# rasmusab/bayes.js

Measured on AMD Instinct MI355X. Metric: posterior draws/sec (= param-updates/sec), higher is better.
Workload: dtype f64

## Files before the change

### bayes.js_amd/csrc/amwg_models.h

```cpp
#pragma once
#include "amwg_div.h"
#include "amwg_ld.h"
#include "amwg_pass.h"
#include "amwg_twoval.h"
#include "amwg_types.h"
#include "amwg_window.h"

namespace amwg {

__device__ __forceinline__ double norm_const_sd(double v, double m, double c_sd, double den, double y_hi, double y_lo, int den_ok) {
  const double t = v - m;
  const double tt = t * t;
  const double q = (den_ok && wide_range(tt)) ? div_by_invariant(tt, den, Reciprocal{y_hi, y_lo}) : tt / den;
  return c_sd - q;
}

struct NormCache {
  double sd, c, den;
  Reciprocal y;
  bool den_ok;
};
__device__ __forceinline__ NormCache norm_cache_init() { return NormCache{__builtin_nan(""), 0.0, 0.0, Reciprocal{0.0, 0.0}, false}; }
AMWG_HD NormCache norm_cache_make(double sd, double neg_half_log_2pi) {
  NormCache k;
  k.sd = sd;
  k.c = norm_c(neg_half_log_2pi, sd);
  k.den = norm_den(sd);
  k.y = make_reciprocal(k.den);
  k.den_ok = mid_range(k.den);
  return k;
}
struct NormCacheA { double c, den; };
AMWG_HD_OUTLINE NormCacheA norm_cache_cold_a(double sd, double neg_half_log_2pi) { return NormCacheA{norm_c(neg_half_log_2pi, sd), norm_den(sd)}; }
AMWG_HD_OUTLINE Reciprocal norm_cache_cold_b(double den) { return make_reciprocal(den); }
template <bool COLD = false>
__device__ __forceinline__ void norm_cache_update(NormCache &k, double sd, double neg_half_log_2pi) {
  if (sd != k.sd) {
    if constexpr (COLD) {
      const NormCacheA a = norm_cache_cold_a(sd, neg_half_log_2pi);
      k.sd = sd; k.c = a.c; k.den = a.den;
      k.y = norm_cache_cold_b(a.den);
      k.den_ok = mid_range(a.den);
    } else {
      k = norm_cache_make(sd, neg_half_log_2pi);
    }
  }
}



struct NormalModel {
  static constexpr bool kSplitPrior = false;
  static constexpr bool kUser = false, kHasFast = true, kOneLanePass = false;
  static constexpr int kDerived = 0;
  static constexpr bool kHasBinary = false;
  static constexpr int kMaxThreads = 1024;
  static constexpr int kUnroll = 8;
  struct Pass { double mu, c, den; Reciprocal y; bool fast; const double *x; };
  static constexpr size_t kOneLaneTileLimit = 96 * 1024;
  __host__ __device__ static size_t one_lane_tile_bytes(int n_obs) { return (size_t)n_obs * 8 <= kOneLaneTileLimit ? (size_t)n_obs * 8 : 0; }
  __host__ __device__ static size_t lds_bytes(int n_obs, int, int lanes) { return lanes == 1 ? 0 : (size_t)n_obs * 8; }
  static constexpr bool kDynamicLds = true;
  __host__ __device__ static size_t lds_bytes_of(const DataRef &d, int lanes, int) { return lanes == 1 ? (d.pad > 0 ? one_lane_tile_bytes(d.n_obs) : 0) : (size_t)d.n_obs * 8; }
  __device__ static void stage(unsigned char *smem, const DataRef &d, int tid, int nt, int lanes) {
    if (lanes == 1 && lds_bytes_of(d, 1, nt) == 0) return;
    double *dst = reinterpret_cast<double *>(smem);
    for (int i = tid; i < d.n_obs; i += nt) dst[i] = d.x[i];
  }
  template <class C>
  __device__ __forceinline__ static double prior(const StateView &, const ModelConsts &mc, const DataRef &, C &kc) {
    double lp = 0;
    lp += norm_const_sd(kc.mu, mc.m0, mc.c0, mc.den0, mc.y0_hi, mc.y0_lo, mc.den0_ok);
    const double sigma = kc.sigma;
    lp += (sigma < mc.ua || sigma > mc.ub) ? -kInf : mc.lunif;
    return lp;
  }
  static constexpr bool kTracksState = true;
  struct Cache { NormCache n; double mu, sigma; bool loaded; };
  __device__ __forceinline__ static Cache cache_init() { return Cache{norm_cache_init(), 0.0, 0.0, false}; }
  __device__ __forceinline__ static void on_set(Cache &k, int comp, double v, int, const DataRef &) { k.mu = comp == 0 ? v : k.mu; k.sigma = comp == 0 ? k.sigma : v; }
  static constexpr bool kMirrorCheck = true;
  template <int GL>
  __device__ __forceinline__ static bool mirror_ok(const Cache &k, const StateView &S, const DataRef &, int) {
    return !k.loaded || (f64_bits(k.mu) == f64_bits(S(0)) && f64_bits(k.sigma) == f64_bits(S(1)));
  }
  template <int GL>
  __device__ __forceinline__ static void load(Cache &k, const StateView &S, const ModelConsts &, const DataRef &, const unsigned char *, int) {
    if (!k.loaded) { k.mu = S(0); k.sigma = S(1); k.loaded = true; }
  }
  template <int GL>
  __device__ __forceinline__ static Pass begin(const StateView &, const ModelConsts &mc, const DataRef &d,
                                               const unsigned char *smem, Cache &kc) {
    Pass ps;
    NormCache &k = kc.n;
    ps.mu = kc.mu;
    norm_cache_update(k, kc.sigma, mc.neg_half_log_2pi);
    ps.c = k.c;
    ps.den = k.den;
    ps.y = k.y;
    ps.fast = !mc.exact_division && mc.data_mid_range && k.den_ok &&
              (ps.mu == 0 || mid_range(__builtin_fabs(ps.mu)));
    ps.x = GL == 1 ? d.x : reinterpret_cast<const double *>(smem);
    return ps;
  }
  template <bool FAST>
  __device__ __forceinline__ static double term(const Pass &ps, int i) {
    const double t = ps.x[i] - ps.mu;
    const double tt = t * t;
    return ps.c - (FAST ? div_by_invariant(tt, ps.den, ps.y) : tt / ps.den);
  }
  template <int G>
  __device__ inline __attribute__((noinline)) static double pass_slow_impl(const double *x, double mu, double c, double den, int n_obs, int sub, double acc) {
    for (int i = sub; i < n_obs; i += G) { const double t = x[i] - mu; acc += c - (t * t) / den; }
    return acc;
  }
  template <int G>
  __device__ __forceinline__ static double pass_slow(const Pass &ps, int n_obs, int sub, double acc) { return pass_slow_impl<G>(ps.x, ps.mu, ps.c, ps.den, n_obs, sub, acc); }
  static constexpr bool kStagedFast = true;
  template <int G, int U = 8>
  __device__ __forceinline__ static double pass_fast(const Pass &ps, int n_obs, int sub, double acc) {
    if constexpr (G == 1) return norm_pass_uniform<8>(ps.x, ps.mu, ps.c, ps.den, ps.y, n_obs, acc);
    else return norm_pass_staged<G, U, false>(ps.x, nullptr, StateView{nullptr}, ps.mu, ps.c, ps.den, ps.y, n_obs, sub, acc);
  }
  static constexpr bool kCertified = true;
  static constexpr int kCertifiedLanes = 1;
  struct Approx { double value, eps; };
  template <int G, int BT>
  __device__ __forceinline__ static Approx log_post_approx(Cache &kc, const StateView &S, const ModelConsts &mc, const DataRef &d, const unsigned char *smem, int sub) {
    static_assert(G == 1, "the certified pass of the Normal family is the one-lane one");
    load<G>(kc, S, mc, d, smem, sub);
    norm_cache_update(kc.n, kc.sigma, mc.neg_half_log_2pi);
    const double P = prior(S, mc, d, kc);
    double S2;
    if (mc.sufficient) {
      const double dm = (mc.suff_xbar_hi - kc.mu) + mc.suff_xbar_lo;
      S2 = __builtin_fma((double)d.n_obs, dm * dm, mc.suff_ss);
    } else
    if constexpr (BT <= 512) S2 = norm_sq_pass_wave<(BT <= 256 ? kWaveBlock : 8)>(lds_bytes_of(d, 1, 0) ? reinterpret_cast<const double *>(smem) : d.x, kc.mu, d.n_obs, wave_scratch_of(d));
    else S2 = norm_sq_pass_uniform<8>(d.x, kc.mu, d.n_obs);
    const double n = (double)d.n_obs;
    const double Q = S2 * kc.n.y.hi, nc = n * kc.n.c;
    const double mag = __builtin_fabs(P) + __builtin_fabs(nc) + 2.0 * Q;
    return Approx{(P + nc) - Q, (2.0 * n + 64.0) * 0x1p-53 * mag * 1.25};
  }
};

struct BetaBernModel {
  static constexpr bool kSplitPrior = false;
  static constexpr bool kUser = false, kHasFast = false, kOneLanePass = true;
  static constexpr int kDerived = 0;
  static constexpr bool kHasBinary = false;
  static constexpr int kMaxThreads = 1024;
  static constexpr int kUnroll = 8;
  struct Pass { double l1, l0; const uint8_t *x; const uint32_t *bits; bool has_invalid, fast_forward; BitData B; };
  __host__ __device__ static size_t words(int n_obs) { return (size_t)n_obs / 32 + 2; }
  static constexpr size_t kFfLdsLimit = 120 * 1024;
  __host__ __device__ static size_t lds_bytes(int n_obs, int, int lanes) {
    if (lanes == 1) { const size_t b = 6 * words(n_obs) * 4; return b <= kFfLdsLimit ? ((b + 15) & ~(size_t)15) : 0; }
    return ((size_t)n_obs + 15) & ~(size_t)15;
  }
  __device__ static void stage(unsigned char *smem, const DataRef &d, int tid, int nt, int lanes) {
    if (lanes == 1) {
      if (lds_bytes(d.n_obs, 0, 1) == 0) return;
      uint32_t *dst = reinterpret_cast<uint32_t *>(smem);
      const uint32_t *src = static_cast<const uint32_t *>(d.arr[0]);
      for (int k = tid; k < (int)(6 * words(d.n_obs)); k += nt) dst[k] = src[k];
      return;
    }
    for (int i = tid; i < d.n_obs; i += nt) smem[i] = d.xb[i];
  }
  template <class C>
  __device__ __forceinline__ static double prior(const StateView &S, const ModelConsts &mc, const DataRef &, C &) {
    const double th = S(0);
    double lp = 0;
    if (th > 1 || th < 0) lp += -kInf;
    else if (mc.ba == 1 && mc.bb == 1) lp += 0.0;
    else lp += (mc.ba - 1) * log_v8(th) + (mc.bb - 1) * log_v8(1 - th) - mc.lbeta_ab;
    return lp;
  }
  struct Cache {};
  __device__ __forceinline__ static Cache cache_init() { return Cache{}; }
  template <int GL>
  __device__ __forceinline__ static Pass begin(const StateView &S, const ModelConsts &mc, const DataRef &d,
                                               const unsigned char *smem, Cache &) {
    Pass ps;
    const double th = S(0);
    ps.l1 = log_v8(th);
    ps.l0 = log_v8(1 - th);
    ps.x = smem;
    ps.bits = d.xw;
    ps.has_invalid = mc.has_invalid != 0;
    ps.fast_forward = !mc.exact_division;
    {
      const size_t W = words(d.n_obs);
      const uint32_t *base = lds_bytes(d.n_obs, 0, 1) ? reinterpret_cast<const uint32_t *>(smem) : static_cast<const uint32_t *>(d.arr[0]);
      ps.B.w = base; ps.B.pre = base + W; ps.B.om1 = base + 2 * W; ps.B.po1 = base + 3 * W; ps.B.om0 = base + 4 * W; ps.B.po0 = base + 5 * W;
      ps.B.n = d.n_obs;
    }
    return ps;
  }
  template <bool FAST>
  __device__ __forceinline__ static double term(const Pass &ps, int i) { return ps.x[i] ? ps.l1 : ps.l0; }

#define AMWG_A0 "v_add_f64 %[acc], %[acc], %[l0]\n"
#define AMWG_A1 "v_add_f64 %[acc], %[acc], %[l1]\n"
#define AMWG_N0 AMWG_A0 AMWG_A0 AMWG_A0 AMWG_A0
#define AMWG_N1 AMWG_A1 AMWG_A0 AMWG_A0 AMWG_A0
#define AMWG_N2 AMWG_A0 AMWG_A1 AMWG_A0 AMWG_A0
#define AMWG_N3 AMWG_A1 AMWG_A1 AMWG_A0 AMWG_A0
#define AMWG_N4 AMWG_A0 AMWG_A0 AMWG_A1 AMWG_A0
#define AMWG_N5 AMWG_A1 AMWG_A0 AMWG_A1 AMWG_A0
#define AMWG_N6 AMWG_A0 AMWG_A1 AMWG_A1 AMWG_A0
#define AMWG_N7 AMWG_A1 AMWG_A1 AMWG_A1 AMWG_A0
#define AMWG_N8 AMWG_A0 AMWG_A0 AMWG_A0 AMWG_A1
#define AMWG_N9 AMWG_A1 AMWG_A0 AMWG_A0 AMWG_A1
#define AMWG_N10 AMWG_A0 AMWG_A1 AMWG_A0 AMWG_A1
#define AMWG_N11 AMWG_A1 AMWG_A1 AMWG_A0 AMWG_A1
#define AMWG_N12 AMWG_A0 AMWG_A0 AMWG_A1 AMWG_A1
#define AMWG_N13 AMWG_A1 AMWG_A0 AMWG_A1 AMWG_A1
#define AMWG_N14 AMWG_A0 AMWG_A1 AMWG_A1 AMWG_A1
#define AMWG_N15 AMWG_A1 AMWG_A1 AMWG_A1 AMWG_A1
#define AMWG_B(HI, LO) AMWG_N##LO AMWG_N##HI "s_branch 25b\n"
#define AMWG_ROW(HI)                                                                                   \
  AMWG_B(HI, 0) AMWG_B(HI, 1) AMWG_B(HI, 2) AMWG_B(HI, 3) AMWG_B(HI, 4) AMWG_B(HI, 5) AMWG_B(HI, 6) AMWG_B(HI, 7) \
  AMWG_B(HI, 8) AMWG_B(HI, 9) AMWG_B(HI, 10) AMWG_B(HI, 11) AMWG_B(HI, 12) AMWG_B(HI, 13) AMWG_B(HI, 14) AMWG_B(HI, 15)
#define AMWG_BERN_ADD_BIT0                                                                             \
  asm volatile("s_bitcmp1_b32 %3, 0\n\ts_cbranch_scc1 1f\n\tv_add_f64 %0, %0, %2\n\ts_branch 2f\n"        \
               "1:\n\tv_add_f64 %0, %0, %1\n2:"                                                        \
               : "+v"(acc) : "v"(l1), "v"(l0), "s"(w) : "scc")
  __device__ __forceinline__ static double pass_one_lane(const Pass &ps, int n_obs, double acc) {
    if (ps.fast_forward) return two_valued_sum(acc, ps.l1, ps.l0, ps.B);
    return pass_one_lane_sequential(ps, n_obs, acc);
  }
  __device__ __attribute__((noinline)) static double pass_one_lane_sequential(const Pass &ps, int n_obs, double acc) {
    const double l1 = ps.l1, l0 = ps.l0;
    const uint64_t pbits = (uint64_t)reinterpret_cast<uintptr_t>(ps.bits);
    const uint32_t plo = __builtin_amdgcn_readfirstlane((uint32_t)pbits), phi = __builtin_amdgcn_readfirstlane((uint32_t)(pbits >> 32));
    const uint32_t *bits = reinterpret_cast<const uint32_t *>((uintptr_t)(((uint64_t)phi << 32) | plo));
    n_obs = __builtin_amdgcn_readfirstlane(n_obs);
    const int nw = n_obs >> 5;
    if (nw > 0) {
      asm volatile(
          "s_mov_b64 s[40:41], %[ptr]\n"
          "s_mov_b32 s42, %[nw]\n"
          "s_getpc_b64 s[44:45]\n"
          "10:\n"
          "s_add_u32 s44, s44, 30f-10b\n"
          "s_addc_u32 s45, s45, 0\n"
          "20:\n"
          "s_load_dword s46, s[40:41], 0x0\n"
          "s_mov_b32 s47, 1\n"
          "s_add_u32 s40, s40, 4\n"
          "s_addc_u32 s41, s41, 0\n"
          "s_waitcnt lgkmcnt(0)\n"
          "22:\n"
          "s_and_b32 s48, s46, 0xff\n"
          "s_mul_i32 s48, s48, 68\n"
          "s_add_u32 s48, s44, s48\n"
          "s_addc_u32 s49, s45, 0\n"
          "s_setpc_b64 s[48:49]\n"
          "25:\n"
          "s_lshr_b64 s[46:47], s[46:47], 8\n"
          "s_cmp_lg_u64 s[46:47], 1\n"
          "s_cbranch_scc1 22b\n"
          "s_sub_u32 s42, s42, 1\n"
          "s_cmp_lg_u32 s42, 0\n"
          "s_cbranch_scc1 20b\n"
          "s_branch 40f\n"
          "30:\n"
          AMWG_ROW(0) AMWG_ROW(1) AMWG_ROW(2) AMWG_ROW(3) AMWG_ROW(4) AMWG_ROW(5) AMWG_ROW(6) AMWG_ROW(7)
          AMWG_ROW(8) AMWG_ROW(9) AMWG_ROW(10) AMWG_ROW(11) AMWG_ROW(12) AMWG_ROW(13) AMWG_ROW(14) AMWG_ROW(15)
          "40:\n"
          : [acc] "+v"(acc)
          : [l1] "v"(l1), [l0] "v"(l0), [ptr] "s"(bits), [nw] "s"(nw)
          : "s40", "s41", "s42", "s44", "s45", "s46", "s47", "s48", "s49", "scc", "memory");
    }
    if (n_obs & 31) {
      uint32_t w = __builtin_amdgcn_readfirstlane(bits[nw]);
      for (int b = 0; b < (n_obs & 31); ++b) {
        AMWG_BERN_ADD_BIT0;
        w >>= 1;
      }
    }
    return acc;
  }
#undef AMWG_BERN_ADD_BIT0
#undef AMWG_ROW
#undef AMWG_B
};

struct HierNormalModel {
  static constexpr bool kUser = false, kHasFast = true, kOneLanePass = false;
  static constexpr int kDerived = 0;
  static constexpr bool kHasBinary = false;
  static constexpr int kMaxThreads = 1024;
  static constexpr int kUnroll = 8;
  struct Pass { double c, den, th_pass; Reciprocal y; bool fast, lane_const, regs, rows; const double *x; const uint8_t *g; StateView S; };
  __host__ __device__ static size_t lds_bytes(int n_obs, int, int) { return (size_t)n_obs * 8 + (((size_t)n_obs + 15) & ~(size_t)15); }
  static constexpr int kMaxLocal = 4;
  __host__ __device__ static int row_pitch(int n_obs) { return ((n_obs + 63) / 64) | 1; }
  __host__ __device__ static int local_rows(int groups) { const int per_group = groups > 0 ? 64 / groups : 1; const int r = per_group < 2 ? 2 : per_group; return r > kMaxLocal ? kMaxLocal : r; }
  __host__ __device__ static int term_pitch(int pitch) { return (pitch + 16 + 1) & ~1; }
  __host__ __device__ static size_t rows_window_offset(int pitch, int waves, int groups) { return (size_t)64 * pitch * 8 + 64 + (size_t)waves * local_rows(groups) * term_pitch(pitch) * 8; }
  __host__ __device__ static size_t rows_lds_bytes(int pitch, int waves, int groups) { return rows_window_offset(pitch, waves, groups) + (size_t)waves * 256 * 8; }
  using SweepStream = WindowStream;
  __device__ __forceinline__ static size_t window_offset(const DataRef &d, int waves) { return rows_window_offset(d.pad, waves, d.G); }
  __device__ __forceinline__ static int sweep_base(const DataRef &) { return 0; }
  __device__ __forceinline__ static int sweep_len(const DataRef &d) { return d.G; }
  __device__ __forceinline__ static int sweep_comp(const unsigned char *smem, const DataRef &d, int sub) {
    return sub < d.G ? sub : (sub < d.n_obs ? (int)(smem + (size_t)64 * d.pad * 8)[sub] : -1);
  }
  static constexpr bool kDynamicLds = true;
  __host__ __device__ static size_t lds_bytes_of(const DataRef &d, int lanes, int threads) { return d.pad > 0 ? rows_lds_bytes(d.pad, threads / 64, d.G) : lds_bytes(d.n_obs, d.G, lanes); }
  __device__ static void stage(unsigned char *smem, const DataRef &d, int tid, int nt, int) {
    double *dst = reinterpret_cast<double *>(smem);
    if (d.pad > 0) {
      const int Rp = d.pad;
      for (int i = tid; i < d.n_obs; i += nt) dst[(i & 63) * Rp + (i >> 6)] = d.x[i];
      uint8_t *gd = smem + (size_t)64 * Rp * 8;
      for (int i = tid; i < 64; i += nt) gd[i] = i < d.n_obs ? d.xb[i] : 0;
      return;
    }
    uint8_t *gd = smem + (size_t)d.n_obs * 8;
    for (int i = tid; i < d.n_obs; i += nt) { dst[i] = d.x[i]; gd[i] = d.xb[i]; }
  }
  static constexpr bool kSplitPrior = true;
  static constexpr bool kTracksState = true;
  struct Cache {
    NormCache n; double th_own, th_pass, mu, sigma; int my_group; bool regs, loaded;
    double pr_mu, pr_sigma, pr_val, c1, den1, y1h, y1l; int den1_ok;
    double a_start, a_mean, a_sd, a_T, b_start, b_mean, b_sd, b_T;
    bool a_recent;
    double s2, s2_mean;
  };
  __device__ __forceinline__ static Cache cache_init() {
    const double nan = __builtin_nan("");
    return Cache{norm_cache_init(), 0.0, 0.0, 0.0, 0.0, -1, false, false, nan, nan, 0.0, 0.0, 0.0, 0.0, 0.0, 0, nan, nan, nan, 0.0, nan, nan, nan, 0.0, false, 0.0, nan};
  }
  template <int GL>
  __device__ __forceinline__ static void load(Cache &k, const StateView &S, const ModelConsts &mc, const DataRef &d, const unsigned char *smem, int sub) {
    if (k.loaded) return;
    constexpr int L = GL < 64 ? GL : 64;
    k.loaded = true;
    k.regs = mc.group_lane_const != 0 && d.G <= L;
    const int j = sub & (L - 1);
    k.mu = S(d.G);
    k.sigma = S(d.G + 1);
    k.my_group = (k.regs && sub < d.n_obs) ? (int)(smem + (d.pad > 0 ? (size_t)64 * d.pad * 8 : (size_t)d.n_obs * 8))[sub] : -1;
    k.th_own = (k.regs && j < d.G) ? S(j) : 0.0;
    k.th_pass = k.my_group >= 0 ? S(k.my_group) : 0.0;
    k.c1 = mc.c1; k.den1 = mc.den1; k.y1h = mc.y1_hi; k.y1l = mc.y1_lo; k.den1_ok = mc.den1_ok;
#if defined(__HIP_DEVICE_COMPILE__)
    asm volatile("" : "+v"(k.c1), "+v"(k.den1), "+v"(k.y1h), "+v"(k.y1l), "+v"(k.den1_ok));
#endif
  }
  __device__ inline __attribute__((noinline)) static double prior_mu_sigma_impl(double mu, double sigma, double m0, double c0, double den0, double y0h, double y0l, int den0_ok,
                                                                                 double ua, double ub, double lunif) {
    double lp = 0;
    lp += norm_const_sd(mu, m0, c0, den0, y0h, y0l, den0_ok);
    lp += (sigma < ua || sigma > ub) ? -kInf : lunif;
    return lp;
  }
  __device__ __forceinline__ static double prior_mu_sigma_cold(double mu, double sigma) {
    const cold_args_ptr ca = cold_args();
    return prior_mu_sigma_impl(mu, sigma, ca->mc.m0, ca->mc.c0, ca->mc.den0, ca->mc.y0_hi, ca->mc.y0_lo, ca->mc.den0_ok, ca->mc.ua, ca->mc.ub, ca->mc.lunif);
  }
  __device__ __forceinline__ static void on_set(Cache &k, int comp, double v, int sub, const DataRef &d) {
    k.th_own = (comp == (sub & 63)) ? v : k.th_own;
    k.th_pass = (comp == k.my_group) ? v : k.th_pass;
    k.mu = (comp == d.G) ? v : k.mu;
    k.sigma = (comp == d.G + 1) ? v : k.sigma;
  }
  static constexpr bool kMirrorCheck = true;
  template <int GL>
  __device__ __forceinline__ static bool mirror_ok(const Cache &k, const StateView &S, const DataRef &d, int sub) {
    if (!k.loaded) return true;
    constexpr int L = GL < 64 ? GL : 64;
    const int j = sub & (L - 1);
    bool ok = f64_bits(k.mu) == f64_bits(S(d.G)) && f64_bits(k.sigma) == f64_bits(S(d.G + 1));
    if (k.regs) {
      if (j < d.G) ok = ok && f64_bits(k.th_own) == f64_bits(S(j));
      if (k.my_group >= 0) ok = ok && f64_bits(k.th_pass) == f64_bits(S(k.my_group));
    }
    return ok;
  }
  template <class C>
  __device__ __forceinline__ static double prior(const StateView &, const ModelConsts &mc, const DataRef &, C &k) {
    const double mu = k.mu, sigma = k.sigma;
#if defined(__HIP_DEVICE_COMPILE__)
    if (mu != k.pr_mu || sigma != k.pr_sigma) { k.pr_mu = mu; k.pr_sigma = sigma; k.pr_val = prior_mu_sigma_cold(mu, sigma); }
    return k.pr_val;
#else
    double lp = 0;
    lp += norm_const_sd(mu, mc.m0, mc.c0, mc.den0, mc.y0_hi, mc.y0_lo, mc.den0_ok);
    lp += (sigma < mc.ua || sigma > mc.ub) ? -kInf : mc.lunif;
    return lp;
#endif
  }
  template <int G, class C>
  __device__ __forceinline__ static double prior_split(const StateView &S, const ModelConsts &mc, const DataRef &d, int sub, double acc, C &k) {
    const double mu = k.mu;
    if (k.regs) {
      if (sub < d.G) acc += norm_const_sd(k.th_own, mu, k.c1, k.den1, k.y1h, k.y1l, k.den1_ok);
      return acc;
    }
    for (int q = sub; q < d.G; q += G) acc += norm_const_sd(S(q), mu, mc.c1, mc.den1, mc.y1_hi, mc.y1_lo, mc.den1_ok);
    return acc;
  }
  template <int GL>
  __device__ __forceinline__ static Pass begin(const StateView &S, const ModelConsts &mc, const DataRef &d,
                                               const unsigned char *smem, Cache &k) {
    Pass ps;
    NormCache &kc = k.n;
    norm_cache_update<true>(kc, k.sigma, mc.neg_half_log_2pi);
    ps.c = kc.c;
    ps.den = kc.den;
    ps.y = kc.y;
    bool ok = !mc.exact_division && mc.data_mid_range && kc.den_ok;
    {
      constexpr int L = GL < 64 ? GL : 64;
      const int lane = (int)(threadIdx.x & 63u), sub_in_wave = lane & (L - 1);
      bool mine = true;
#if defined(AMWG_X_CUT_BEGIN)
      if (k.regs) { }
#else
      if (k.regs) { if (sub_in_wave < d.G) { const double th = k.th_own; mine = th == 0 || mid_range(__builtin_fabs(th)); } }
#endif
      else for (int q = sub_in_wave; q < d.G; q += L) { const double th = S(q); mine = mine && (th == 0 || mid_range(__builtin_fabs(th))); }
      if constexpr (L == 1) ok = ok && mine;
      else {
        const uint64_t all = __ballot(mine);
        const uint64_t group = (L == 64 ? ~0ull : ((1ull << (L & 63)) - 1ull)) << (lane & ~(L - 1));
        ok = ok && ((all & group) == group);
      }
    }
    ps.fast = ok;
    ps.x = reinterpret_cast<const double *>(smem);
    ps.g = smem + (size_t)d.n_obs * 8;
    ps.S = S;
    ps.lane_const = mc.group_lane_const != 0;
    ps.regs = k.regs;
// ... 585 lines not shown
```

### bayes.js_amd/csrc/amwg_pass.h

```cpp
#pragma once
#include "amwg_div.h"
#include "amwg_types.h"

namespace amwg {

#if defined(__HIP_DEVICE_COMPILE__)
#define AMWG_STAGE_FENCE() __builtin_amdgcn_sched_barrier(0)
#else
#define AMWG_STAGE_FENCE() ((void)0)
#endif

template <int U>
struct NormBlock { double v[U]; };

#if defined(__HIP_DEVICE_COMPILE__)
#define AMWG_WAIT_LDS_LE(n) __builtin_amdgcn_s_waitcnt(0xC07F | ((n) << 8))
#else
#define AMWG_WAIT_LDS_LE(n) ((void)0)
#endif

template <int U, bool ADD_PREV>
AMWG_HD void norm_block_stages(NormBlock<U> &b, const double (&m)[U], NormBlock<U> &q, const NormBlock<U> &prev, double &acc,
                                                  double c, double den, Reciprocal y) {
  int a = 0;
  auto add_prev = [&](int upto) {
    if constexpr (ADD_PREV) { for (; a < upto && a < U; ++a) acc = acc + prev.v[a]; }
  };
#pragma unroll
  for (int u = 0; u < U; ++u) b.v[u] = b.v[u] - m[u];
  add_prev(1 * U / 7);
  AMWG_STAGE_FENCE();
#pragma unroll
  for (int u = 0; u < U; ++u) b.v[u] = b.v[u] * b.v[u];
  add_prev(2 * U / 7);
  AMWG_STAGE_FENCE();
#pragma unroll
  for (int u = 0; u < U; ++u) q.v[u] = b.v[u] * y.lo;
  add_prev(3 * U / 7);
  AMWG_STAGE_FENCE();
#pragma unroll
  for (int u = 0; u < U; ++u) q.v[u] = __builtin_fma(b.v[u], y.hi, q.v[u]);
  add_prev(4 * U / 7);
  AMWG_STAGE_FENCE();
#pragma unroll
  for (int u = 0; u < U; ++u) b.v[u] = __builtin_fma(-den, q.v[u], b.v[u]);
  add_prev(5 * U / 7);
  AMWG_STAGE_FENCE();
#pragma unroll
  for (int u = 0; u < U; ++u) q.v[u] = __builtin_fma(b.v[u], y.hi, q.v[u]);
  add_prev(6 * U / 7);
  AMWG_STAGE_FENCE();
#pragma unroll
  for (int u = 0; u < U; ++u) q.v[u] = c - q.v[u];
  add_prev(U);
  AMWG_STAGE_FENCE();
}

template <int G, int U, bool GATHER, class XT = double>
AMWG_HD double norm_pass_staged(const XT *x, const uint8_t *g, const StateView S, double mean, double c, double den,
                                                   Reciprocal y, int n_obs, int sub, double acc) {
  const int n_full = n_obs / G, rem = n_obs % G;
  const int n_blocks = n_full / U;
  int k = 0;
  if (n_blocks > 0) {
    NormBlock<U> xa, xb, qa, qb;
    double ma[U], mb[U];
    int ga[U], gb[U];
    const XT *px = x + sub;
    const uint8_t *pg = g + sub;
    auto load_idx = [&](int blk, int (&gi)[U]) {
      if constexpr (GATHER) {
        blk = blk < n_blocks ? blk : n_blocks - 1;
#pragma unroll
        for (int u = 0; u < U; ++u) gi[u] = pg[(blk * U + u) * G];
      }
    };
    auto load_val = [&](int blk, NormBlock<U> &xv, double (&mv)[U], const int (&gi)[U]) {
#pragma unroll
      for (int u = 0; u < U; ++u) xv.v[u] = (double)px[(blk * U + u) * G];
#pragma unroll
      for (int u = 0; u < U; ++u) mv[u] = GATHER ? S(gi[u]) : mean;
    };
    load_idx(0, ga);
    load_val(0, xa, ma, ga);
    load_idx(1, gb);
    AMWG_STAGE_FENCE();
    if (n_blocks > 1) { load_val(1, xb, mb, gb); load_idx(2, ga); }
    AMWG_STAGE_FENCE();
    norm_block_stages<U, false>(xa, ma, qa, qa, acc, c, den, y);
    int blk = 1;
    for (; blk + 2 < n_blocks; blk += 2) {
      load_val(blk + 1, xa, ma, ga);
      load_idx(blk + 2, gb);
      AMWG_STAGE_FENCE();
      if constexpr (!GATHER && U == 8 && sizeof(XT) == 8) { AMWG_WAIT_LDS_LE(4); AMWG_STAGE_FENCE(); }
      norm_block_stages<U, true>(xb, mb, qb, qa, acc, c, den, y);
      load_val(blk + 2, xb, mb, gb);
      load_idx(blk + 3, ga);
      AMWG_STAGE_FENCE();
      if constexpr (!GATHER && U == 8 && sizeof(XT) == 8) { AMWG_WAIT_LDS_LE(4); AMWG_STAGE_FENCE(); }
      norm_block_stages<U, true>(xa, ma, qa, qb, acc, c, den, y);
    }
    if (blk < n_blocks) {
      if (blk + 1 < n_blocks) load_val(blk + 1, xa, ma, ga);
      AMWG_STAGE_FENCE();
      norm_block_stages<U, true>(xb, mb, qb, qa, acc, c, den, y);
      if (blk + 1 < n_blocks) {
        norm_block_stages<U, true>(xa, ma, qa, qb, acc, c, den, y);
#pragma unroll
        for (int u = 0; u < U; ++u) acc = acc + qa.v[u];
      } else {
#pragma unroll
        for (int u = 0; u < U; ++u) acc = acc + qb.v[u];
      }
    } else {
#pragma unroll
      for (int u = 0; u < U; ++u) acc = acc + qa.v[u];
    }
    k = n_blocks * U;
  }
  const int left = n_full - k;
  if (left + (rem > 0 ? 1 : 0) <= U / 2 + 1) {
    constexpr int TMAX = U / 2 + 1;
    double xv[TMAX], mv[TMAX];
    const int cnt_all = left + (rem > 0 ? 1 : 0);
    if (cnt_all > 0) {
#pragma unroll
    for (int r = 0; r < TMAX; ++r) {
      int i = (k + (r < cnt_all ? r : 0)) * G + sub;
      i = i < n_obs ? i : n_obs - 1;
      xv[r] = (double)x[i];
      mv[r] = GATHER ? S(g[i]) : mean;
    }
    AMWG_STAGE_FENCE();
#pragma unroll
    for (int r = 0; r < TMAX; ++r) {
      if (r < cnt_all) {
        const double t = xv[r] - mv[r];
        const double term = c - div_by_invariant(t * t, den, y);
        const bool mine = r < left || sub < rem;
        acc = mine ? acc + term : acc;
      }
    }
    }
  } else if (left > 0 || rem > 0) {
    const int cnt = left + (sub < rem ? 1 : 0);
    NormBlock<U> xt, qt;
    double mt[U];
#pragma unroll
    for (int u = 0; u < U; ++u) {
      int r = u < cnt ? u : (cnt > 0 ? cnt - 1 : 0);
      int i = (k + r) * G + sub;
      i = i < n_obs ? i : n_obs - 1;
      xt.v[u] = (double)x[i];
      mt[u] = GATHER ? S(g[i]) : mean;
    }
    AMWG_STAGE_FENCE();
    norm_block_stages<U, false>(xt, mt, qt, qt, acc, c, den, y);
#pragma unroll
    for (int u = 0; u < U; ++u) acc = u < cnt ? acc + qt.v[u] : acc;
  }
  return acc;
}

#if defined(__HIP_DEVICE_COMPILE__)
typedef const double __attribute__((address_space(4))) *amwg_uniform_f64_ptr;
#else
typedef const double *amwg_uniform_f64_ptr;
#endif

struct StagedFirst { static constexpr bool value = true; };
struct StagedLater { static constexpr bool value = false; };

template <int U>
AMWG_HD double norm_pass_uniform(const double *x_global, double mean, double c, double den, Reciprocal y, int n_obs, double acc) {
  constexpr int CH = 2 * U;
  const int n_chunks = n_obs / CH;
  int k = 0;
  if (n_chunks > 0) {
    amwg_uniform_f64_ptr px = (amwg_uniform_f64_ptr)(uintptr_t)x_global;
    double ma[U];
#pragma unroll
    for (int u = 0; u < U; ++u) ma[u] = mean;
    NormBlock<CH> sa, sb;
    NormBlock<U> ta, tb, qa, qb;
    auto load_chunk = [&](int ch, NormBlock<CH> &dst) {
      ch = ch < n_chunks ? ch : n_chunks - 1;
#pragma unroll
      for (int u = 0; u < CH; ++u) dst.v[u] = px[ch * CH + u];
    };
    auto lo = [&](const NormBlock<CH> &src, NormBlock<U> &t) {
#pragma unroll
      for (int u = 0; u < U; ++u) t.v[u] = src.v[u];
    };
    auto hi = [&](const NormBlock<CH> &src, NormBlock<U> &t) {
#pragma unroll
      for (int u = 0; u < U; ++u) t.v[u] = src.v[U + u];
    };
    auto compute = [&](const NormBlock<CH> &src, auto first) {
      lo(src, ta);
      norm_block_stages<U, !decltype(first)::value>(ta, ma, qa, qb, acc, c, den, y);
      hi(src, tb);
      norm_block_stages<U, true>(tb, ma, qb, qa, acc, c, den, y);
    };
    load_chunk(0, sb);
    AMWG_WAIT_LDS_LE(0); AMWG_STAGE_FENCE();
    load_chunk(1, sa);
    AMWG_STAGE_FENCE();
    compute(sb, StagedFirst{});
    int ch = 1;
    for (; ch + 1 < n_chunks; ch += 2) {
      AMWG_WAIT_LDS_LE(0); AMWG_STAGE_FENCE();
      load_chunk(ch + 1, sb);
      AMWG_STAGE_FENCE();
      compute(sa, StagedLater{});
      AMWG_WAIT_LDS_LE(0); AMWG_STAGE_FENCE();
      load_chunk(ch + 2, sa);
      AMWG_STAGE_FENCE();
      compute(sb, StagedLater{});
    }
    if (ch < n_chunks) {
      AMWG_WAIT_LDS_LE(0); AMWG_STAGE_FENCE();
      compute(sa, StagedLater{});
    }
#pragma unroll
    for (int u = 0; u < U; ++u) acc = acc + qb.v[u];
    k = n_chunks * CH;
  }
  for (; k < n_obs; ++k) {
    const double t = x_global[k] - mean;
    acc += c - div_by_invariant(t * t, den, y);
  }
  return acc;
}

template <int U>
AMWG_HD double norm_sq_pass_uniform(const double *x_global, double mean, int n_obs) {
  constexpr int CH = 2 * U;
  double acc[U];
#pragma unroll
  for (int u = 0; u < U; ++u) acc[u] = 0.0;
  const int n_chunks = n_obs / CH;
  int k = 0;
  if (n_chunks > 0) {
    amwg_uniform_f64_ptr px = (amwg_uniform_f64_ptr)(uintptr_t)x_global;
    NormBlock<CH> sa, sb;
    auto load_chunk = [&](int ch, NormBlock<CH> &dst) {
      ch = ch < n_chunks ? ch : n_chunks - 1;
#pragma unroll
      for (int u = 0; u < CH; ++u) dst.v[u] = px[ch * CH + u];
    };
    auto compute = [&](const NormBlock<CH> &src) {
#pragma unroll
      for (int u = 0; u < U; ++u) { const double t = src.v[u] - mean; acc[u] = __builtin_fma(t, t, acc[u]); }
      AMWG_STAGE_FENCE();
#pragma unroll
      for (int u = 0; u < U; ++u) { const double t = src.v[U + u] - mean; acc[u] = __builtin_fma(t, t, acc[u]); }
      AMWG_STAGE_FENCE();
    };
    load_chunk(0, sb);
    AMWG_WAIT_LDS_LE(0); AMWG_STAGE_FENCE();
    load_chunk(1, sa);
    AMWG_STAGE_FENCE();
    compute(sb);
    int ch = 1;
    for (; ch + 1 < n_chunks; ch += 2) {
      AMWG_WAIT_LDS_LE(0); AMWG_STAGE_FENCE();
      load_chunk(ch + 1, sb);
      AMWG_STAGE_FENCE();
      compute(sa);
      AMWG_WAIT_LDS_LE(0); AMWG_STAGE_FENCE();
      load_chunk(ch + 2, sa);
      AMWG_STAGE_FENCE();
      compute(sb);
    }
    if (ch < n_chunks) {
      AMWG_WAIT_LDS_LE(0); AMWG_STAGE_FENCE();
      compute(sa);
    }
    k = n_chunks * CH;
  }
  for (; k < n_obs; ++k) {
    const double t = x_global[k] - mean;
    acc[0] = __builtin_fma(t, t, acc[0]);
  }
  double s = 0.0;
#pragma unroll
  for (int u = 0; u < U; ++u) s += acc[u];
  return s;
}

#if defined(__HIPCC__) || defined(__HIPCC_RTC__)
#ifndef AMWG_WAVE_BLOCK
#define AMWG_WAVE_BLOCK 16
#endif
constexpr int kWaveBlock = AMWG_WAVE_BLOCK;
template <int N> struct PassBlock { static constexpr int value = N; };
typedef int amwg_v16i __attribute__((ext_vector_type(16)));
__device__ __forceinline__ double *wave_scratch_of(const DataRef &d) {
#if defined(__HIP_DEVICE_COMPILE__)
  if (!d.wave_scratch) return nullptr;
  const uint32_t wave = (uint32_t)__builtin_amdgcn_readfirstlane((int)(blockIdx.x * (blockDim.x >> 6) + (threadIdx.x >> 6)));
  return d.wave_scratch + (size_t)wave * 64;
#else
  (void)d; return nullptr;
#endif
}
template <int B>
__device__ __forceinline__ double norm_sq_pass_wave(const double *x, double mu, int n_obs, double *scr = nullptr) {
#if defined(__HIP_DEVICE_COMPILE__)
  const int lane = (int)(threadIdx.x & 63u);
  double a[64];
#pragma unroll
  for (int c = 0; c < 64; ++c) a[c] = 0.0;
  const int mu_lo = (int)(uint32_t)f64_bits(mu), mu_hi = (int)(uint32_t)(f64_bits(mu) >> 32);
  auto mean_of = [&](int c) { return bits_f64(((uint64_t)(uint32_t)__builtin_amdgcn_readlane(mu_hi, c) << 32) | (uint64_t)(uint32_t)__builtin_amdgcn_readlane(mu_lo, c)); };
  bool smem_done = false;
#if !defined(AMWG_X_NO_SMEM_MEANS)
  if (scr != nullptr) {
    scr[lane] = mu;
    asm volatile("s_waitcnt vmcnt(0)\n\ts_dcache_inv\n\ts_waitcnt lgkmcnt(0)" ::: "memory");
    auto fetch = [&](int g) { amwg_v16i r; asm volatile("s_load_dwordx16 %0, %1, %2" : "=&s"(r) : "s"(scr), "s"(g * 8)); return r; };
    auto landed = [&](amwg_v16i &r) { asm volatile("s_waitcnt lgkmcnt(0)" : "+s"(r)); };
    auto mean_in = [&](const amwg_v16i &r, int j) { return bits_f64(((uint64_t)(uint32_t)r[2 * j + 1] << 32) | (uint64_t)(uint32_t)r[2 * j]); };
    auto block_s = [&](auto tag, int at) {
      constexpr int BB = decltype(tag)::value;
      double xv[BB];
      amwg_v16i cur = fetch(0);
#pragma unroll
      for (int b = 0; b < BB; ++b) xv[b] = x[at + b * 64 + lane];
#pragma unroll
      for (int g = 0; g < 64; g += 8) {
        landed(cur);
        amwg_v16i nxt = cur;
        if (g + 8 < 64) nxt = fetch(g + 8);
#pragma unroll
        for (int b = 0; b < BB; ++b) {
#pragma unroll
          for (int j = 0; j < 8; ++j) { const double t = xv[b] - mean_in(cur, j); a[g + j] = __builtin_fma(t, t, a[g + j]); }
        }
        cur = nxt;
      }
    };
    int base = 0;
    for (; base + 64 * B <= n_obs; base += 64 * B) block_s(PassBlock<B>{}, base);
    if constexpr (B >= 32) { if (base + 64 * 16 <= n_obs) { block_s(PassBlock<16>{}, base); base += 64 * 16; } }
    if constexpr (B >= 16) { if (base + 64 * 8 <= n_obs) { block_s(PassBlock<8>{}, base); base += 64 * 8; } }
    if constexpr (B >= 8) { if (base + 64 * 4 <= n_obs) { block_s(PassBlock<4>{}, base); base += 64 * 4; } }
    if constexpr (B >= 4) { if (base + 64 * 2 <= n_obs) { block_s(PassBlock<2>{}, base); base += 64 * 2; } }
    for (; base + 64 <= n_obs; base += 64) block_s(PassBlock<1>{}, base);
    if (base < n_obs) {
      const int i = base + lane;
      const bool has = i < n_obs;
      const double xv = x[has ? i : base];
      amwg_v16i cur = fetch(0);
#pragma unroll
      for (int g = 0; g < 64; g += 8) {
        landed(cur);
        amwg_v16i nxt = cur;
        if (g + 8 < 64) nxt = fetch(g + 8);
#pragma unroll
        for (int j = 0; j < 8; ++j) { const double t = has ? xv - mean_in(cur, j) : 0.0; a[g + j] = __builtin_fma(t, t, a[g + j]); }
        cur = nxt;
      }
    }
    smem_done = true;
  }
#endif
  if (!smem_done) {
  auto block = [&](auto tag, int at) {
    constexpr int BB = decltype(tag)::value;
    double xv[BB];
#pragma unroll
    for (int b = 0; b < BB; ++b) xv[b] = x[at + b * 64 + lane];
#pragma unroll
    for (int g = 0; g < 64; g += 8) {
      double m[8];
#pragma unroll
      for (int j = 0; j < 8; ++j) m[j] = mean_of(g + j);
#pragma unroll
      for (int b = 0; b < BB; ++b) {
#pragma unroll
        for (int j = 0; j < 8; ++j) { const double t = xv[b] - m[j]; a[g + j] = __builtin_fma(t, t, a[g + j]); }
      }
    }
  };
  int base = 0;
  for (; base + 64 * B <= n_obs; base += 64 * B) block(PassBlock<B>{}, base);
  if constexpr (B >= 32) { if (base + 64 * 16 <= n_obs) { block(PassBlock<16>{}, base); base += 64 * 16; } }
  if constexpr (B >= 16) { if (base + 64 * 8 <= n_obs) { block(PassBlock<8>{}, base); base += 64 * 8; } }
  if constexpr (B >= 8) { if (base + 64 * 4 <= n_obs) { block(PassBlock<4>{}, base); base += 64 * 4; } }
  if constexpr (B >= 4) { if (base + 64 * 2 <= n_obs) { block(PassBlock<2>{}, base); base += 64 * 2; } }
  if constexpr (B >= 2) { if (base + 64 <= n_obs) { block(PassBlock<1>{}, base); base += 64; } }
  for (; base + 64 <= n_obs; base += 64) block(PassBlock<1>{}, base);
  if (base < n_obs) {
    const int i = base + lane;
    const bool has = i < n_obs;
    const double xv = x[has ? i : base];
#pragma unroll
    for (int g = 0; g < 64; g += 8) {
      double m[8];
#pragma unroll
      for (int j = 0; j < 8; ++j) m[j] = mean_of(g + j);
#pragma unroll
      for (int j = 0; j < 8; ++j) { const double t = has ? xv - m[j] : 0.0; a[g + j] = __builtin_fma(t, t, a[g + j]); }
    }
  }
  }
  auto swap_add = [&](double A, double Bv, int off) {
    const uint32_t al = (uint32_t)f64_bits(A), ah = (uint32_t)(f64_bits(A) >> 32), bl = (uint32_t)f64_bits(Bv), bh = (uint32_t)(f64_bits(Bv) >> 32);
    if (off == 32) {
      const auto l = __builtin_amdgcn_permlane32_swap(al, bl, false, false), h = __builtin_amdgcn_permlane32_swap(ah, bh, false, false);
      return bits_f64(((uint64_t)h[0] << 32) | (uint64_t)l[0]) + bits_f64(((uint64_t)h[1] << 32) | (uint64_t)l[1]);
    } else {
      const auto l = __builtin_amdgcn_permlane16_swap(al, bl, false, false), h = __builtin_amdgcn_permlane16_swap(ah, bh, false, false);
      return bits_f64(((uint64_t)h[0] << 32) | (uint64_t)l[0]) + bits_f64(((uint64_t)h[1] << 32) | (uint64_t)l[1]);
    }
  };
#pragma unroll
  for (int j = 0; j < 32; ++j) a[j] = swap_add(a[j], a[j + 32], 32);
#pragma unroll
  for (int j = 0; j < 16; ++j) a[j] = swap_add(a[j], a[j + 16], 16);
  {
    const bool up = (lane & 8) != 0;
#pragma unroll
    for (int j = 0; j < 8; ++j) { const double send = up ? a[j] : a[j + 8], keep = up ? a[j + 8] : a[j]; a[j] = keep + xor_partner<8, true>(send); }
  }
  {
    const bool up = (lane & 4) != 0;
#pragma unroll
    for (int j = 0; j < 4; ++j) { const double send = up ? a[j] : a[j + 4], keep = up ? a[j + 4] : a[j]; a[j] = keep + xor_partner<4, true>(send); }
  }
  {
    const bool up = (lane & 2) != 0;
#pragma unroll
    for (int j = 0; j < 2; ++j) { const double send = up ? a[j] : a[j + 2], keep = up ? a[j + 2] : a[j]; a[j] = keep + xor_partner<2>(send); }
  }
  {
    const bool up = (lane & 1) != 0;
    const double send = up ? a[0] : a[1], keep = up ? a[1] : a[0];
    a[0] = keep + xor_partner<1>(send);
  }
  return a[0];
#else
  (void)x; (void)mu; (void)n_obs;
  return 0.0;
#endif
}
#endif

}
```

### bayes.js_amd/csrc/amwg_user.h

```cpp
#pragma once
#include "amwg_div.h"
#include "amwg_ld.h"
#include "amwg_pass.h"
#include "amwg_twoval.h"
#include "amwg_kval.h"
#include "amwg_types.h"

namespace amwg {

template <int J>
AMWG_HD const void *user_arr(const DataRef &d) {
  if constexpr (J < kInlineUserArrays) return d.arr[J];
  else return d.arr_ext[J - kInlineUserArrays];
}

struct NormInv { double c, den; Reciprocal y; bool fast; };
AMWG_HD NormInv norm_inv(double sd) {
  NormInv k;
  k.c = norm_c(-0.5 * log_v8(2 * kPi), sd);
  k.den = norm_den(sd);
  k.y = make_reciprocal(k.den);
  k.fast = mid_range(k.den);
  return k;
}
AMWG_HD double ld_norm_inv(double x, double mean, const NormInv &k) {
  const double t = x - mean;
  const double tt = t * t;
  const double q = (k.fast && wide_range(tt)) ? div_by_invariant(tt, k.den, k.y) : tt / k.den;
  return k.c - q;
}

AMWG_HD double ld_norm_fast(double x, double mean, const NormInv &k, uint32_t &rlo, uint32_t &rhi) {
  const double t = x - mean;
  const double tt = t * t;
  const uint32_t h = (uint32_t)hi_word(tt);
  rlo = h < rlo ? h : rlo;
  rhi = h > rhi ? h : rhi;
  return k.c - div_by_invariant(tt, k.den, k.y);
}
AMWG_HD double ld_norm_slow(double x, double mean, const NormInv &k) {
  const double t = x - mean;
  return k.c - (t * t) / k.den;
}
AMWG_HD bool norm_range_ok(uint32_t rlo, uint32_t rhi) { return rlo >= 0x1A700000u && rhi <= 0x65700000u; }

template <class T, class U> struct SameType { static constexpr bool value = false; };
template <class T> struct SameType<T, T> { static constexpr bool value = true; };
template <int G, class XT>
AMWG_HD double norm_data_loop(const XT *x_staged, const XT *x_global, int n, double mean, const NormInv &k, bool data_mid_range, int sub, double acc) {
  if (k.fast && data_mid_range && (mean == 0 || mid_range(__builtin_fabs(mean)))) {
#if defined(__HIP_DEVICE_COMPILE__)
    if constexpr (G == 1 && SameType<XT, double>::value) return norm_pass_uniform<8>(x_global, mean, k.c, k.den, k.y, n, acc);
    else return norm_pass_staged<G, 8, false, XT>(x_staged, nullptr, StateView{nullptr}, mean, k.c, k.den, k.y, n, sub, acc);
#else
    for (int i = sub; i < n; i += G) { const double t = (double)x_global[i] - mean; acc += k.c - div_by_invariant(t * t, k.den, k.y); }
    return acc;
#endif
  }
  const XT *x = (G == 1 && SameType<XT, double>::value) ? x_global : x_staged;
  for (int i = sub; i < n; i += G) { const double t = (double)x[i] - mean; acc += k.c - (t * t) / k.den; }
  return acc;
}

struct TailApprox { double value, eps; };
#if defined(__HIPCC__) || defined(__HIPCC_RTC__)
template <class M, int G, int BT>
__device__ __forceinline__ TailApprox norm_tail_approx(const StateView &S, const DataRef &d, const unsigned char *smem, int sub) {
  static_assert(G == 1, "the certified tail of a translated closure is the one-lane one");
#if defined(__HIP_DEVICE_COMPILE__)
  const double head = M::template tail_head<1>(S, d, smem, 0);
  const NormInv k = norm_inv(M::tail_sd(S, d));
  const double mean = M::tail_mean(S, d);
  double S2;
  if constexpr (BT <= 256) S2 = norm_sq_pass_wave<kWaveBlock>(M::tail_x(d, smem), mean, M::kTailN, wave_scratch_of(d));
  else S2 = norm_sq_pass_uniform<8>(M::tail_x_global(d), mean, M::kTailN);
  const double n = (double)M::kTailN;
  const double Q = S2 * k.y.hi, nc = n * k.c;
  const double mag = __builtin_fabs(head) + __builtin_fabs(nc) + 2.0 * Q;
  return TailApprox{(head + nc) - Q, (2.0 * n + 64.0) * 0x1p-53 * mag * 1.25};
#else
  (void)S; (void)d; (void)smem; (void)sub;
  return TailApprox{0.0, __builtin_inf()};
#endif
}
#endif

template <int G, bool PERIODIC, class XT>
AMWG_HD double norm_data_loop_gather(const XT *x, const uint8_t *g, const StateView &S, int base, int n_groups, int n, const NormInv &k,
                                     bool data_mid_range, int sub, double acc) {
  bool ok = k.fast && data_mid_range;
#if defined(__HIP_DEVICE_COMPILE__)
  {
    constexpr int L = G < 64 ? G : 64;
    const int lane = (int)(threadIdx.x & 63u);
    bool mine = true;
    for (int j = lane & (L - 1); j < n_groups; j += L) { const double th = S(base + j); mine = mine && (th == 0 || mid_range(__builtin_fabs(th))); }
    if constexpr (L == 1) ok = ok && mine;
    else {
      const uint64_t all = __ballot(mine);
      const uint64_t group = (L == 64 ? ~0ull : ((1ull << (L & 63)) - 1ull)) << (lane & ~(L - 1));
      ok = ok && ((all & group) == group);
    }
  }
  if (ok) {
    const StateView T{S.base + base};
    if constexpr (PERIODIC) {
      const double m = sub < n ? T(g[sub]) : 0.0;
      return norm_pass_staged<G, 8, false, XT>(x, nullptr, T, m, k.c, k.den, k.y, n, sub, acc);
    } else {
      return norm_pass_staged<G, 4, true, XT>(x, g, T, 0.0, k.c, k.den, k.y, n, sub, acc);
    }
  }
#else
  for (int j = 0; j < n_groups; ++j) { const double th = S(base + j); ok = ok && (th == 0 || mid_range(__builtin_fabs(th))); }
  if (ok) {
    for (int i = sub; i < n; i += G) { const double t = (double)x[i] - S(base + g[i]); acc += k.c - div_by_invariant(t * t, k.den, k.y); }
    return acc;
  }
#endif
  for (int i = sub; i < n; i += G) { const double t = (double)x[i] - S(base + g[i]); acc += k.c - (t * t) / k.den; }
  return acc;
}

struct BernInv { double l1, l0; };
AMWG_HD BernInv bern_inv(double p) { return BernInv{ld_bern(1.0, p), ld_bern(0.0, p)}; }
AMWG_HD double ld_bern_inv(double x, const BernInv &k) { return x == 1 ? k.l1 : (x == 0 ? k.l0 : -kInf); }
template <class T> AMWG_HD double ld_bern_inv01(T x, const BernInv &k) { return x != 0 ? k.l1 : k.l0; }

AMWG_HD double ld_pois_pre(double x, double lambda, double lfact_x) { return x < 0 ? -kInf : log_v8(lambda) * x - lambda - lfact_x; }
AMWG_HD double ld_pois_pre_exp(double x, double eta, double lfact_x) {
  double lambda;
  const double lg = exp_log_v8(eta, lambda, ExpLogLiterals{});
  return x < 0 ? -kInf : lg * x - lambda - lfact_x;
}
AMWG_HD double ld_pois_exp(double x, double eta) {
  double lambda;
  const double lg = exp_log_v8(eta, lambda, ExpLogLiterals{});
  return x < 0 ? -kInf : lg * x - lambda - lfactorial_js(x);
}
AMWG_HD double ld_binom_pre(double x, double size, double prob, double lchoose_size_x) {
  if (x > size || x < 0) return -kInf;
  if (prob == 0 || prob == 1) return (size * prob) == x ? 0.0 : -kInf;
  return lchoose_size_x + x * log_v8(prob) + (size - x) * log_v8(1 - prob);
}

AMWG_HD double bern_loop_one_lane(double acc, const BernInv &k, const int32_t *tab, int n) {
  const size_t W = two_valued_words(n);
  const uint32_t *t = reinterpret_cast<const uint32_t *>(tab);
  const BitData B{t, t + W, t + 2 * W, t + 3 * W, t + 4 * W, t + 5 * W, n};
  return two_valued_sum(acc, k.l1, k.l0, B);
}

template <int K>
AMWG_HD double kval_loop_one_lane(double acc, const double (&c)[K], const int32_t *tab, const uint8_t *idx, int n) {
  const KValData B{reinterpret_cast<const uint32_t *>(tab), idx, n};
  return k_valued_sum<K>(acc, c, B);
}

AMWG_HD double js_mod(double a, double b) {
  const uint64_t ua = f64_bits(a), ub = f64_bits(b);
  const uint64_t sign = ua & 0x8000000000000000ull;
  uint64_t ma = ua & 0x7fffffffffffffffull, mb = ub & 0x7fffffffffffffffull;
  if (ma >= 0x7ff0000000000000ull || mb > 0x7ff0000000000000ull || mb == 0) return __builtin_nan("");
  if (ma < mb) return a;
  if (ma == mb) return bits_f64(sign);
  int ea = (int)(ma >> 52), eb = (int)(mb >> 52);
  if (ea == 0) { const int sh = __builtin_clzll(ma) - 11; ma <<= sh; ea = 1 - sh; }
  else ma = (ma & 0x000fffffffffffffull) | 0x0010000000000000ull;
  if (eb == 0) { const int sh = __builtin_clzll(mb) - 11; mb <<= sh; eb = 1 - sh; }
  else mb = (mb & 0x000fffffffffffffull) | 0x0010000000000000ull;
  for (; ea > eb; --ea) {
    if (ma >= mb) ma -= mb;
    ma <<= 1;
  }
  if (ma >= mb) ma -= mb;
  if (ma == 0) return bits_f64(sign);
  const int sh = __builtin_clzll(ma) - 11;
  ma <<= sh;
  ea -= sh;
  if (ea > 0) ma = (ma & 0x000fffffffffffffull) | ((uint64_t)ea << 52);
  else ma >>= (1 - ea);
  return bits_f64(ma | sign);
}
AMWG_HD double js_max(double a, double b) {
  if (a != a || b != b) return __builtin_nan("");
  if (a == b) return (a == 0 && __builtin_signbit(a)) ? b : a;
  return a > b ? a : b;
}
AMWG_HD double js_min(double a, double b) {
  if (a != a || b != b) return __builtin_nan("");
  if (a == b) return (a == 0 && __builtin_signbit(a)) ? a : b;
  return a < b ? a : b;
}
AMWG_HD double js_sign(double x) { return x > 0 ? 1.0 : (x < 0 ? -1.0 : x); }
AMWG_HD double js_trunc(double x) { return __builtin_trunc(x); }
AMWG_HD int32_t js_toint32(double x) {
  if (!(__builtin_fabs(x) < __builtin_inf())) return 0;
  const double t = __builtin_trunc(x);
  if (t >= -2147483648.0 && t <= 2147483647.0) return (int32_t)t;
  double m = js_mod(t, 4294967296.0);
  if (m < 0) m += 4294967296.0;
  return (int32_t)(uint32_t)m;
}
AMWG_HD double js_bitor(double a, double b) { return (double)(js_toint32(a) | js_toint32(b)); }
AMWG_HD double js_bitand(double a, double b) { return (double)(js_toint32(a) & js_toint32(b)); }
AMWG_HD double js_bitxor(double a, double b) { return (double)(js_toint32(a) ^ js_toint32(b)); }
AMWG_HD double js_bitnot(double a) { return (double)(~js_toint32(a)); }
AMWG_HD double js_shl(double a, double b) { return (double)(int32_t)((uint32_t)js_toint32(a) << ((uint32_t)js_toint32(b) & 31u)); }
AMWG_HD double js_shr(double a, double b) { return (double)(js_toint32(a) >> ((uint32_t)js_toint32(b) & 31u)); }
AMWG_HD double js_ushr(double a, double b) { return (double)((uint32_t)js_toint32(a) >> ((uint32_t)js_toint32(b) & 31u)); }
AMWG_HD double js_imul(double a, double b) { return (double)(int32_t)((uint32_t)js_toint32(a) * (uint32_t)js_toint32(b)); }
AMWG_HD double js_clz32(double a) { const uint32_t u = (uint32_t)js_toint32(a); return u == 0 ? 32.0 : (double)__builtin_clz(u); }
AMWG_HD double js_fround(double a) { return (double)(float)a; }

}

#include "amwg_rows.h"
#include "amwg_ptail.h"
#include "amwg_ltail.h"
```

Baseline: 1.429 billion.

## Software-pipeline wave sum-of-squares pass with LDS-typed pointer and row prefetch

Restructures the wave-level squared-deviation pass so the next block's data rows are prefetched into registers in two halves while the current block is computed, and per-chain means are fetched once and double-buffered across blocks. Adds an LDS address-space pointer path so tiled data is read with LDS instructions, and replaces the cascaded tail blocks with bitmask-driven partial-row reads. This aims to hide memory and scalar-load latency behind the FMA work, at the cost of more register pressure and more complex tail handling. The code also references M::kTailXLds, which is not defined anywhere in the shown code.

```diff
diff --git a/bayes.js_amd/csrc/amwg_models.h b/bayes.js_amd/csrc/amwg_models.h
--- a/bayes.js_amd/csrc/amwg_models.h
+++ b/bayes.js_amd/csrc/amwg_models.h
@@ -136,7 +136,13 @@
       const double dm = (mc.suff_xbar_hi - kc.mu) + mc.suff_xbar_lo;
       S2 = __builtin_fma((double)d.n_obs, dm * dm, mc.suff_ss);
     } else
-    if constexpr (BT <= 512) S2 = norm_sq_pass_wave<(BT <= 256 ? kWaveBlock : 8)>(lds_bytes_of(d, 1, 0) ? reinterpret_cast<const double *>(smem) : d.x, kc.mu, d.n_obs, wave_scratch_of(d));
+    if constexpr (BT <= 512) {
+      constexpr int B = BT <= 256 ? kWaveBlock : 8;
+      double *scr = wave_scratch_of(d);
+      const bool tile = lds_bytes_of(d, 1, 0) != 0;
+      if (tile && scr != nullptr) S2 = norm_sq_pass_wave<B, true>((amwg_lds_f64_ptr)smem, kc.mu, d.n_obs, scr);
+      else S2 = norm_sq_pass_wave<B>(tile ? reinterpret_cast<const double *>(smem) : d.x, kc.mu, d.n_obs, scr);
+    }
     else S2 = norm_sq_pass_uniform<8>(d.x, kc.mu, d.n_obs);
     const double n = (double)d.n_obs;
     const double Q = S2 * kc.n.y.hi, nc = n * kc.n.c;
diff --git a/bayes.js_amd/csrc/amwg_pass.h b/bayes.js_amd/csrc/amwg_pass.h
--- a/bayes.js_amd/csrc/amwg_pass.h
+++ b/bayes.js_amd/csrc/amwg_pass.h
@@ -290,6 +290,10 @@
   return s;
 }
 
+struct PassRows { int blocks, full, masked; };
+AMWG_HD PassRows pass_rows(int n_obs, int B) { const int rows = n_obs / 64; return PassRows{rows / B, rows % B, (n_obs % 64) != 0 ? 1 : 0}; }
+AMWG_HD constexpr int pass_part_slot(int B, int p) { return B - 2 * p; }
+AMWG_HD constexpr int pass_part_row(int full, int p) { return full & ~(2 * p - 1); }
 #if defined(__HIPCC__) || defined(__HIPCC_RTC__)
 #ifndef AMWG_WAVE_BLOCK
 #define AMWG_WAVE_BLOCK 16
@@ -306,10 +310,16 @@
   (void)d; return nullptr;
 #endif
 }
-template <int B>
-__device__ __forceinline__ double norm_sq_pass_wave(const double *x, double mu, int n_obs, double *scr = nullptr) {
-#if defined(__HIP_DEVICE_COMPILE__)
-  const int lane = (int)(threadIdx.x & 63u);
+#if defined(__HIP_DEVICE_COMPILE__)
+typedef const double __attribute__((address_space(3))) *amwg_lds_f64_ptr;
+#else
+typedef const double *amwg_lds_f64_ptr;
+#endif
+template <int B, bool SCALAR_ONLY = false, class XP = const double *>
+__device__ __forceinline__ double norm_sq_pass_wave(XP x, double mu, int n_obs, double *scr = nullptr) {
+#if defined(__HIP_DEVICE_COMPILE__)
+  int lane = (int)(threadIdx.x & 63u);
+  asm volatile("" : "+v"(lane));
   double a[64];
 #pragma unroll
   for (int c = 0; c < 64; ++c) a[c] = 0.0;
@@ -317,57 +327,90 @@
   auto mean_of = [&](int c) { return bits_f64(((uint64_t)(uint32_t)__builtin_amdgcn_readlane(mu_hi, c) << 32) | (uint64_t)(uint32_t)__builtin_amdgcn_readlane(mu_lo, c)); };
   bool smem_done = false;
 #if !defined(AMWG_X_NO_SMEM_MEANS)
-  if (scr != nullptr) {
+  if (SCALAR_ONLY || scr != nullptr) {
+    const PassRows pr = pass_rows(n_obs, B);
+    double xv[B];
+    auto read_rows = [&](int blk, int b0, int b1) {
+#pragma unroll
+      for (int b = b0; b < b1; ++b) xv[b] = x[(blk * B + b) * 64 + lane];
+    };
+    if (pr.blocks > 0) read_rows(0, 0, B);
     scr[lane] = mu;
     asm volatile("s_waitcnt vmcnt(0)\n\ts_dcache_inv\n\ts_waitcnt lgkmcnt(0)" ::: "memory");
     auto fetch = [&](int g) { amwg_v16i r; asm volatile("s_load_dwordx16 %0, %1, %2" : "=&s"(r) : "s"(scr), "s"(g * 8)); return r; };
     auto landed = [&](amwg_v16i &r) { asm volatile("s_waitcnt lgkmcnt(0)" : "+s"(r)); };
     auto mean_in = [&](const amwg_v16i &r, int j) { return bits_f64(((uint64_t)(uint32_t)r[2 * j + 1] << 32) | (uint64_t)(uint32_t)r[2 * j]); };
-    auto block_s = [&](auto tag, int at) {
-      constexpr int BB = decltype(tag)::value;
-      double xv[BB];
-      amwg_v16i cur = fetch(0);
-#pragma unroll
-      for (int b = 0; b < BB; ++b) xv[b] = x[at + b * 64 + lane];
+    amwg_v16i cur = fetch(0);
+    landed(cur);
+    auto rows_s = [&](auto r0, auto rn, auto refill) {
+      constexpr int R0 = decltype(r0)::value, RN = decltype(rn)::value, RH = R0 + RN / 2;
 #pragma unroll
       for (int g = 0; g < 64; g += 8) {
-        landed(cur);
-        amwg_v16i nxt = cur;
-        if (g + 8 < 64) nxt = fetch(g + 8);
-#pragma unroll
-        for (int b = 0; b < BB; ++b) {
+        amwg_v16i nxt = fetch(g + 8 < 64 ? g + 8 : 0);
+        AMWG_STAGE_FENCE();
+#pragma unroll
+        for (int b = R0; b < RH; ++b) {
 #pragma unroll
           for (int j = 0; j < 8; ++j) { const double t = xv[b] - mean_in(cur, j); a[g + j] = __builtin_fma(t, t, a[g + j]); }
         }
+        if (g + 8 == 64) { AMWG_STAGE_FENCE(); refill(R0, RH); AMWG_STAGE_FENCE(); }
+#pragma unroll
+        for (int b = RH; b < R0 + RN; ++b) {
+#pragma unroll
+          for (int j = 0; j < 8; ++j) { const double t = xv[b] - mean_in(cur, j); a[g + j] = __builtin_fma(t, t, a[g + j]); }
+        }
+        if (g + 8 == 64) AMWG_STAGE_FENCE();
+        landed(nxt);
+        if (g + 8 == 64) { AMWG_STAGE_FENCE(); refill(RH, R0 + RN); AMWG_STAGE_FENCE(); }
         cur = nxt;
       }
     };
-    int base = 0;
-    for (; base + 64 * B <= n_obs; base += 64 * B) block_s(PassBlock<B>{}, base);
-    if constexpr (B >= 32) { if (base + 64 * 16 <= n_obs) { block_s(PassBlock<16>{}, base); base += 64 * 16; } }
-    if constexpr (B >= 16) { if (base + 64 * 8 <= n_obs) { block_s(PassBlock<8>{}, base); base += 64 * 8; } }
-    if constexpr (B >= 8) { if (base + 64 * 4 <= n_obs) { block_s(PassBlock<4>{}, base); base += 64 * 4; } }
-    if constexpr (B >= 4) { if (base + 64 * 2 <= n_obs) { block_s(PassBlock<2>{}, base); base += 64 * 2; } }
-    for (; base + 64 <= n_obs; base += 64) block_s(PassBlock<1>{}, base);
-    if (base < n_obs) {
-      const int i = base + lane;
-      const bool has = i < n_obs;
-      const double xv = x[has ? i : base];
-      amwg_v16i cur = fetch(0);
-#pragma unroll
-      for (int g = 0; g < 64; g += 8) {
-        landed(cur);
-        amwg_v16i nxt = cur;
-        if (g + 8 < 64) nxt = fetch(g + 8);
-#pragma unroll
-        for (int j = 0; j < 8; ++j) { const double t = has ? xv - mean_in(cur, j) : 0.0; a[g + j] = __builtin_fma(t, t, a[g + j]); }
-        cur = nxt;
+    for (int k = 0; k < pr.blocks; ++k) {
+      const int nb = k + 1 < pr.blocks ? k + 1 : k;
+      rows_s(PassBlock<0>{}, PassBlock<B>{}, [&](int b0, int b1) { read_rows(nb, b0, b1); });
+    }
+    if (pr.full > 0 || pr.masked) {
+      const int rbase = pr.blocks * B * 64 + lane;
+      const bool has = pr.masked && rbase + pr.full * 64 < n_obs;
+      auto read_part = [&](auto pt) {
+        constexpr int P = decltype(pt)::value;
+        if (pr.full & P) {
+#pragma unroll
+          for (int b = 0; b < P; ++b) xv[pass_part_slot(B, P) + b] = x[rbase + (pass_part_row(pr.full, P) + b) * 64];
+        }
+      };
+      if constexpr (B >= 32) read_part(PassBlock<16>{});
+      if constexpr (B >= 16) read_part(PassBlock<8>{});
+      if constexpr (B >= 8) read_part(PassBlock<4>{});
+      if constexpr (B >= 4) read_part(PassBlock<2>{});
+      if constexpr (B >= 2) read_part(PassBlock<1>{});
+      if (pr.masked) xv[B - 1] = x[has ? rbase + pr.full * 64 : 0];
+      auto part = [&](auto pt) {
+        constexpr int P = decltype(pt)::value;
+        if (pr.full & P) rows_s(PassBlock<pass_part_slot(B, P)>{}, pt, [](int, int) {});
+      };
+      if constexpr (B >= 32) part(PassBlock<16>{});
+      if constexpr (B >= 16) part(PassBlock<8>{});
+      if constexpr (B >= 8) part(PassBlock<4>{});
+      if constexpr (B >= 4) part(PassBlock<2>{});
+      if constexpr (B >= 2) part(PassBlock<1>{});
+      if (pr.masked) {
+        const double xm = xv[B - 1];
+#pragma unroll
+        for (int g = 0; g < 64; g += 8) {
+          amwg_v16i nxt = cur;
+          if (g + 8 < 64) nxt = fetch(g + 8);
+#pragma unroll
+          for (int j = 0; j < 8; ++j) { const double t = has ? xm - mean_in(cur, j) : 0.0; a[g + j] = __builtin_fma(t, t, a[g + j]); }
+          if (g + 8 < 64) landed(nxt);
+          cur = nxt;
+        }
       }
     }
     smem_done = true;
   }
 #endif
-  if (!smem_done) {
+  if constexpr (!SCALAR_ONLY) if (!smem_done) {
   auto block = [&](auto tag, int at) {
     constexpr int BB = decltype(tag)::value;
     double xv[BB];
diff --git a/bayes.js_amd/csrc/amwg_user.h b/bayes.js_amd/csrc/amwg_user.h
--- a/bayes.js_amd/csrc/amwg_user.h
+++ b/bayes.js_amd/csrc/amwg_user.h
@@ -72,7 +72,12 @@
   const NormInv k = norm_inv(M::tail_sd(S, d));
   const double mean = M::tail_mean(S, d);
   double S2;
-  if constexpr (BT <= 256) S2 = norm_sq_pass_wave<kWaveBlock>(M::tail_x(d, smem), mean, M::kTailN, wave_scratch_of(d));
+  if constexpr (BT <= 256) {
+    double *scr = wave_scratch_of(d);
+    bool done = false;
+    if constexpr (M::kTailXLds) { if (scr != nullptr) { S2 = norm_sq_pass_wave<kWaveBlock, true>((amwg_lds_f64_ptr)M::tail_x(d, smem), mean, M::kTailN, scr); done = true; } }
+    if (!done) S2 = norm_sq_pass_wave<kWaveBlock>(M::tail_x(d, smem), mean, M::kTailN, scr);
+  }
   else S2 = norm_sq_pass_uniform<8>(M::tail_x_global(d), mean, M::kTailN);
   const double n = (double)M::kTailN;
   const double Q = S2 * k.y.hi, nc = n * k.c;
```

Measured after the change: 1.450 billion (median of 6 runs). 1.5% higher.
